# Layjins/Spider

Measured on AMD Instinct MI355X. Metric: multimodal responses/sec (text->text+image), higher is better.
Workload: dtype bf16

## Files before the change

### include/spider_hip.h

```cpp
#ifndef SPIDER_HIP_H
#define SPIDER_HIP_H
#define SPIDER_ABI_VERSION 4

#ifdef __cplusplus
extern "C" {
#endif

int spider_abi_version(void);
const char* spider_target_arch(void);
const char* spider_last_error(void);


int spider_embed_bf16(const void* table, const int* ids, void* out, int rows, int H, int V, void* stream);

int spider_rmsnorm_bf16(const void* x, const void* res, const void* w, void* y, void* res_out, int rows, int H,
                        float eps, void* stream);

int spider_gemv_bf16(const void* W, const void* x, void* out, const void* bias, const void* res, const void* norm_w,
                     float eps, int B, int N, int K, void* stream);

int spider_gemv_swiglu_bf16(const void* W_gate_up, const void* x, void* out, const void* norm_w, float eps, int B,
                            int I, int K, void* stream);

int spider_lm_head_nparts(int V);
// ... 14 lines not shown
int spider_beam_partial_bf16(const void* logits, float* ws_ms, float* ws_val, int* ws_tok, int rows, int V, int C, int nslice,
                             void* stream);
int spider_beam_select_f32(const float* ws_ms, const float* ws_val, const int* ws_tok, float* run_scores, const int* eos_ids,
                           const int* n_eos, const int* n_hist, float* trace_score, int* trace_beam, int* trace_tok, int cap,
                           int* src_beam, int* next_ids, int B, int K, int V, int C, int nslice, void* stream);
int spider_kv_row_gather_bf16(void* k_cache, void* v_cache, void* k_tmp, void* v_tmp, const int* src_beam, const int* kv_beg,
                              const int* kv_end, int K, int R, int layers, int rows_alloc, int n_kv, int T, int d, void* stream);

int spider_sample_partial_bf16(const void* logits, const void* seen, const void* ban, const float* penalty, const int* min_new,
                               const int* eos_ids, const int* n_eos, const int* n_hist, const int* top_k, float* ws_val,
                               int* ws_tok, int rows, int V, int nslice, void* stream);
int spider_sample_select_f32(const float* ws_val, const int* ws_tok, const float* temperature, const float* top_p, const int* top_k,
                             const void* seed, const int* row0, const int* n_hist, int* next_ids, int* cand_tok, float* cand_p,
                             int* n_keep, float* u, int rows, int V, int nslice, void* stream);

int spider_rope_kv_append_bf16(const void* qkv, const int* pos, const int* slot, const float* cos_sin, void* q_out,
                               void* k_cache, void* v_cache, int B, int S, int n_q, int n_kv, int d, int T_max,
                               void* stream);
int spider_rope_kv_append_mrope_bf16(const void* qkv, const int* pos3, const int* slot, const float* cos_sin, void* q_out,
                                     void* k_cache, void* v_cache, int B, int S, int n_q, int n_kv, int d, int T_max,
                                     int sec_t, int sec_h, void* stream);

int spider_attn_decode_bf16(const void* q, const void* k_cache, const void* v_cache, const int* kv_beg,
                            const int* kv_end, void* out, void* ws_o, void* ws_ml, int B, int n_q, int n_kv, int d,
                            int T_max, float scale, int nsplit, void* stream);

int spider_attn_decode_fused_bf16(const void* qkv, const int* pos, const float* cos_sin, void* k_cache, void* v_cache,
                                  const int* kv_beg, const int* kv_end, void* out, void* ws_o, void* ws_ml,
                                  int* counters, int B, int n_q, int n_kv, int d, int T_max, float scale, int nsplit,
                                  void* stream);
int spider_set_attn_inline(int on);
int spider_set_gemv_sched(int sched);
int spider_set_ws_inlaunch(int on);

int spider_gemv_fm_bf16(const void* Wfm, const void* x, void* out, const void* bias, const void* res, int B, int N, int K,
                        int fold_rmsnorm, float eps, void* stream);
int spider_gemv_swiglu_fm_bf16(const void* Wfm_gate_up, const void* x, void* out, int B, int I, int K, int fold_rmsnorm, float eps,
                               void* stream);
int spider_lm_head_argmax_fm_bf16(const void* Wfm, const void* x, int* out_ids, void* logits, void* ws_val, void* ws_idx, int B,
                                  int V, int K, int fold_rmsnorm, float eps, void* stream);
int spider_lm_head_argmax_fm_proc_bf16(const void* Wfm, const void* x, int* out_ids, void* logits, void* ws_val, void* ws_idx,
                                       const void* seen, const void* ban, const float* penalty, const int* min_new,
                                       const int* eos_ids, const int* n_eos, const int* n_hist, int B, int V, int K,
                                       int fold_rmsnorm, float eps, void* stream);


int spider_gemm_bf16(const void* A, const void* W, void* C, void* C32, const void* bias, const void* res,
                     const void* rowbias, int rows_per_group, int M, int N, int K, int lda, int ldc, int act,
                     float out_scale, int w_tiled, const float* res32, float* c32d, void* ws, long ws_bytes, void* stream);

int spider_gemm_ln_bf16(const void* A, const void* Wf, void* C, const float* colsum, const float* colbias, const void* res,
                        int M, int N, int K, int ldc, int act, float eps, int w_tiled, void* ws, long ws_bytes, void* stream);

int spider_xattn_fused_bf16(const void* x, const void* mq_fm, const void* mo_fm, const float* colsum, const float* colbias,
                            const void* bias_o, void* out, int B2, int n_tok, int C, int heads, int n_keys, float eps,
                            const float* x32, float* out32, void* stream);

int spider_conv2d_nhwc_bf16(const void* x, const void* w, void* y, const void* bias, const void* res,
                            const void* rowbias, int B, int Hin, int Win, int Cin, int Cout, int ks, int stride,
                            int pad, int ups, float out_scale, int w_tiled, const float* res32, float* c32d, void* ws, long ws_bytes, void* stream);

int spider_conv_nhwc_ex_bf16(const void* x, const void* w, void* y, const void* bias, const void* res,
                             const void* rowbias, int B, int Hin, int Win, int Cin, int Cout, int kh, int kw, int stride,
                             int pad_h, int pad_w, int dil, int up_h, int up_w, int act, float act_param,
                             float out_scale, int w_tiled, const float* res32, float* c32d, void* ws, long ws_bytes, void* stream);

// ... 181 lines not shown
```

### spider_amd/csrc/capi.cpp

```cpp
#include <string.h>

static thread_local char g_err[512] = "";

extern "C" {

void spider_set_error(const char* msg) {
    strncpy(g_err, msg ? msg : "", sizeof(g_err) - 1);
    g_err[sizeof(g_err) - 1] = 0;
}

const char* spider_last_error(void) { return g_err; }

int spider_abi_version(void) { return 4; }

const char* spider_target_arch(void) { return "gfx950"; }

int g_spider_ws_inlaunch = -1;

int spider_set_ws_inlaunch(int on) {
    const int prev = g_spider_ws_inlaunch;
    g_spider_ws_inlaunch = on ? 1 : 0;
    return prev;
}

}
```

### spider_amd/csrc/common.hpp

```cpp
#pragma once
#include <hip/hip_runtime.h>
#include <stdint.h>

namespace spider {

typedef uint16_t bf16_t;

typedef __attribute__((ext_vector_type(4))) float f32x4;
typedef __attribute__((ext_vector_type(16))) float f32x16;
typedef __attribute__((ext_vector_type(8))) short bf16x8;
typedef __attribute__((ext_vector_type(4))) short bf16x4;

typedef __attribute__((ext_vector_type(4))) uint32_t u32x4;
typedef __attribute__((ext_vector_type(2))) uint32_t u32x2;

__device__ __forceinline__ float bf16_to_f32(bf16_t v) {
    return __uint_as_float(((uint32_t)v) << 16);
}
__device__ __forceinline__ float bf16lo_to_f32(uint32_t packed) {
    return __uint_as_float(packed << 16);
}
__device__ __forceinline__ float bf16hi_to_f32(uint32_t packed) {
    return __uint_as_float(packed & 0xffff0000u);
}
typedef __bf16 hw_bf16x2 __attribute__((ext_vector_type(2)));
typedef float hw_f32x2 __attribute__((ext_vector_type(2)));
__device__ __forceinline__ bf16_t f32_to_bf16(float f) {
    return __builtin_bit_cast(bf16_t, (__bf16)f);
}
__device__ __forceinline__ uint32_t pack_bf16x2(float lo, float hi) {
    const hw_f32x2 v = {lo, hi};
    return __builtin_bit_cast(uint32_t, __builtin_convertvector(v, hw_bf16x2));
}

typedef uint16_t h16_t;
// ... 64 lines not shown
__device__ __forceinline__ float wave_max(float v) {
#pragma unroll
    for (int o = 32; o > 0; o >>= 1) v = fmaxf(v, __shfl_xor(v, o, 64));
    return v;
}

template <int NW>
__device__ __forceinline__ float block_sum(float v, float* red) {
    v = wave_sum(v);
    const int lane = threadIdx.x & 63, w = threadIdx.x >> 6;
    __syncthreads();
    if (lane == 0) red[w] = v;
    __syncthreads();
    float t = 0.f;
#pragma unroll
    for (int i = 0; i < NW; ++i) t += red[i];
    return t;
}

__device__ __forceinline__ float silu_f(float x) { return x * __builtin_amdgcn_rcpf(1.f + __expf(-x)); }
__device__ __forceinline__ float erf_fast(float x) {
    const float ax = fabsf(x);
    const float t = __builtin_amdgcn_rcpf(fmaf(0.3275911f, ax, 1.f));
    float p = fmaf(1.061405429f, t, -1.453152027f);
    p = fmaf(p, t, 1.421413741f);
    p = fmaf(p, t, -0.284496736f);
    p = fmaf(p, t, 0.254829592f);
    const float e = 1.f - p * t * __expf(-ax * ax);
    return copysignf(e, x);
}
__device__ __forceinline__ float gelu_erf_f(float x) { return 0.5f * x * (1.f + erf_fast(x * 0.70710678118654752f)); }
__device__ __forceinline__ float quick_gelu_f(float x) { return x * __builtin_amdgcn_rcpf(1.f + __expf(-1.702f * x)); }

__device__ __forceinline__ int xcd_remap(int bid, int nwg) {
    const int q = nwg >> 3, r = nwg & 7, xcd = bid & 7, idx = bid >> 3;
    const int base = (xcd < r) ? xcd * (q + 1) : r * (q + 1) + (xcd - r) * q;
    return base + idx;
}

}

template <typename F>
inline void raise_dynamic_lds(F* fn, int bytes, unsigned& done_mask) {
    int dev = 0;
    (void)hipGetDevice(&dev);
    const unsigned bit = 1u << (dev & 31);
    if (!(done_mask & bit)) {
        (void)hipFuncSetAttribute(reinterpret_cast<const void*>(fn), hipFuncAttributeMaxDynamicSharedMemorySize, bytes);
        done_mask |= bit;
    }
}

extern "C" void spider_set_error(const char* msg);
extern "C" int g_spider_ws_inlaunch;
#define SPIDER_CHECK(cond, msg)            \
    do {                                   \
        if (!(cond)) {                     \
            spider_set_error(msg);         \
            return -1;                     \
        }                                  \
    } while (0)
#define SPIDER_LAUNCH_OK()                                        \
    do {                                                          \
        hipError_t e__ = hipGetLastError();                       \
        if (e__ != hipSuccess) {                                  \
            spider_set_error(hipGetErrorString(e__));             \
            return -2;                                            \
        }                                                         \
    } while (0)
```

### spider_amd/csrc/gemm.hip

```cpp
#include "common.hpp"
#include <stdlib.h>
#include <stdio.h>
#include <type_traits>

using namespace spider;

namespace {

constexpr int BK = 64;
constexpr int LDS_STRIDE = BK;

struct GemmArgs {
    const h16_t* A;
    const h16_t* W;
    h16_t* C;
    const h16_t* bias;
    const h16_t* res;
    const h16_t* rowbias;
    float* C32;
    const float* res32;
    float* c32d;
    float* ws;
    int M, N, K, lda, ldc;
    uint32_t a_bytes, w_bytes;
    uint32_t c_bytes, rb_bytes;
    int rows_per_group;
    int act;
    float act_param;
    int geglu;
    float out_scale;
    int splits, kt_per_split;
    int conv, Hin, Win, Cin, Hout, Wout, kh, kw, stride, pad_h, pad_w, dil, ups, lim_h, lim_w, cin64;
    int kcm;
    int hbits;
    int dbg;
    int epi_lds;
    int n_fast;
    int w_tiled;
    const float* ln_colsum;
    const float* ln_bias;
    float ln_eps;
    const float2* ln_rows;
    float* gn_part;
    int gn_G, gn_cpg, gn_cr;
    const float* gna_part;
    const h16_t* gna_gamma;
    const h16_t* gna_beta;
    int gna_nchunk, gna_G, gna_hw;
    float gna_eps;
    int ws_ncb, ws_cpb, ws_rows;
    unsigned* ws_cnt;
    int a32;
};

__device__ __forceinline__ float apply_act(const GemmArgs& p, float v) {
    if (p.act == 1) return silu_f(v);
    if (p.act == 2) return gelu_erf_f(v);
    if (p.act == 3) return quick_gelu_f(v);
    if (p.act == 5) return v > 0.f ? v : v * p.act_param;
    if (p.act == 6) return fmaxf(v, 0.f);
    if (p.act == 7) return tanhf(v);
    return v;
}

__device__ __forceinline__ uint32_t w_row_byte(const GemmArgs& p, int n) {
    const uint32_t nk = (uint32_t)((p.K + BK - 1) / BK);
    return p.w_tiled ? ((uint32_t)(n >> 6) * nk * 8192u + (uint32_t)(n & 63) * 128u) : (uint32_t)n * (uint32_t)p.K * 2u;
}
__device__ __forceinline__ uint32_t w_tile_step(const GemmArgs& p) { return p.w_tiled ? 8192u : (uint32_t)(BK * 2); }

// ... 385 lines not shown
        const int m = mb + i * 16 + (lane & 15);
        if (m >= p.M) continue;
#pragma unroll
        for (int j = 0; j < NT; ++j) {
            const int n = nb + j * 16 + (lane >> 4) * 4;
            if (n >= p.N) continue;
            float v[4] = {acc[i][j][0], acc[i][j][1], acc[i][j][2], acc[i][j][3]};
            if (p.splits > 1) {
                float* dst = p.ws + ((size_t)split * p.M + m) * p.N + n;
                if (n + 3 < p.N) *reinterpret_cast<f32x4*>(dst) = f32x4{v[0], v[1], v[2], v[3]};
                else for (int e = 0; e < 4 && n + e < p.N; ++e) dst[e] = v[e];
            } else {
                epilogue_store<EPI>(p, m, n, v);
            }
        }
    }
}

template <int BM, int BN, bool CONV, int EPI, bool LN = false, bool GNA = false, bool A32 = false>
__global__ __launch_bounds__(256, 2) void gemm_kernel(GemmArgs p) {
    constexpr bool GEGLU = EPI == 2;
    extern __shared__ __attribute__((aligned(16))) char smem[];
    h16_t* lds = reinterpret_cast<h16_t*>(smem);
    constexpr int TILE_ELEMS = ((A32 ? 2 : 1) * BM + BN) * LDS_STRIDE;
    constexpr uint32_t AE = A32 ? 4u : 2u;
    constexpr int MT = BM / 32, NT = BN / 32;
    constexpr int AC = BM / 32, WC = BN / 32;

    const int tid = threadIdx.x, lane = tid & 63, wave = tid >> 6;
    const int wm = wave >> 1, wn = wave & 1;

    const int ncols = GEGLU ? 2 * p.N : p.N;
    const int tiles_m = (p.M + BM - 1) / BM, tiles_n = (ncols + BN - 1) / BN;
    const int bid = xcd_remap(blockIdx.x, tiles_m * tiles_n);
    const int tm = p.n_fast ? bid / tiles_n : bid % tiles_m, tn = p.n_fast ? bid % tiles_n : bid / tiles_m;
    const int m0 = tm * BM, n0 = tn * BN;
    const int split = blockIdx.y;

    const int chunk = tid & 7;
    const int lrow = tid >> 3;
    const __amdgpu_buffer_rsrc_t rsrc_a = __builtin_amdgcn_make_buffer_rsrc(const_cast<h16_t*>(p.A), 0, p.a_bytes, 0x00020000);
    const __amdgpu_buffer_rsrc_t rsrc_w = __builtin_amdgcn_make_buffer_rsrc(const_cast<h16_t*>(p.W), 0, p.w_bytes, 0x00020000);
    uint32_t a_base[AC], a_inv[AC];
    uint32_t a_lin[AC];
    uint32_t a_hb[AC];
    int a_oy[AC], a_ox[AC];
    uint32_t w_base[WC], w_inv[WC];
#pragma unroll
    for (int i = 0; i < AC; ++i) {
        const int m = m0 + lrow + 32 * i;
        const bool ok = m < p.M;
        const int mc = ok ? m : 0;
        a_inv[i] = ok ? 0u : 0xFFFFFFFFu;
        if (CONV) {
            const int hw = p.Hout * p.Wout;
            const int b = mc / hw, rem = mc % hw;
            a_oy[i] = (rem / p.Wout) * p.stride - p.pad_h;
            a_ox[i] = (rem % p.Wout) * p.stride - p.pad_w;
            a_base[i] = (uint32_t)b * (uint32_t)(p.Hin * p.Win * p.Cin) * AE;
            a_lin[i] = a_base[i] + (uint32_t)(a_oy[i] * p.Win + a_ox[i]) * (uint32_t)p.Cin * AE;
            a_hb[i] = 0u;
            if (p.hbits) {
                a_lin[i] += chunk * 8u * AE;
                {
                    uint32_t hb = 0u;
                    for (int ky = 0; ky < p.kh; ++ky)
                        for (int kx = 0; kx < p.kw; ++kx) {
                            const int iy = a_oy[i] + ky * p.dil, ix = a_ox[i] + kx * p.dil;
// ... 322 lines not shown
            const int row = idx / CH, c4 = idx - row * CH;
            const int m = m0 + pass * HR + row, n = n0 + c4 * 4;
            const f32x4 q = *reinterpret_cast<const f32x4*>(T + row * LDT + c4 * 4);
            float v[4] = {q[0], q[1], q[2], q[3]};
            uint32_t rb_row = 0;
            if (p.rowbias) rb_row = (uint32_t)((m < p.M ? m : 0) / p.rows_per_group) * (uint32_t)p.N * 2u;
            epilogue_fast<ACT>(p, er, m, n, rb_row, v);
        }
    }
}

template <int N>
__device__ __forceinline__ void wait_vmcnt() {
    asm volatile("s_waitcnt vmcnt(%0)" ::"n"(N) : "memory");
}

template <int BN, int NS, bool CONV, int EPI, int BM = 128, bool GN = false>
__global__ __launch_bounds__(512, NS == 2 ? 2 : 1) void gemm_dma_kernel(GemmArgs p) {
    static_assert(BM == 128 || BM == 64, "row tile");
    constexpr int ROWS = BM + BN;
    constexpr int STAGE = ROWS * 128;
    constexpr int MT = BM / 64, NT = BN / 32;
    constexpr int AJ = BM / 64;
    constexpr int WP = BN / 8;
    constexpr int WJ = (WP + 7) / 8;
    constexpr bool W_RAGGED = (WP % 8) != 0;
    extern __shared__ __attribute__((aligned(16))) char smem[];
    typedef __attribute__((address_space(3))) void* lds_ptr_t;

    const int tid = threadIdx.x, lane = tid & 63;
    const int wave = __builtin_amdgcn_readfirstlane(tid >> 6);
    const int wm = wave >> 1, wn = wave & 1;
    const int tiles_m = (p.M + BM - 1) / BM, tiles_n = (p.N + BN - 1) / BN;
    const int bid = xcd_remap(blockIdx.x, tiles_m * tiles_n);
    const int tm = p.n_fast ? bid / tiles_n : bid % tiles_m, tn = p.n_fast ? bid % tiles_n : bid / tiles_m;
    const int m0 = tm * BM, n0 = tn * BN;
    const int split = blockIdx.y;

    const __amdgpu_buffer_rsrc_t rsrc_a = __builtin_amdgcn_make_buffer_rsrc(const_cast<h16_t*>(p.A), 0, p.a_bytes, 0x00020000);
    const __amdgpu_buffer_rsrc_t rsrc_w = __builtin_amdgcn_make_buffer_rsrc(const_cast<h16_t*>(p.W), 0, p.w_bytes, 0x00020000);

    const int prow = lane >> 3, slot = lane & 7;
    uint32_t a_base[AJ], a_inv[AJ], a_gch[AJ], a_lin[AJ];
    uint32_t a_hb[AJ];
    int a_oy[AJ], a_ox[AJ];
    uint32_t w_base[WJ], w_inv[WJ], w_gch[WJ];
#pragma unroll
    for (int j = 0; j < AJ; ++j) {
        const int R = (j * 8 + wave) * 8 + prow;
        const int m = m0 + R;
        const bool ok = m < p.M;
        const int mc = ok ? m : 0;
        a_gch[j] = (uint32_t)(slot ^ ((R >> 1) & 7));
        a_inv[j] = ok ? 0u : 0xFFFFFFFFu;
        if (CONV) {
            const int hw = p.Hout * p.Wout;
            const int b = mc / hw, rem = mc % hw;
            a_oy[j] = (rem / p.Wout) * p.stride - p.pad_h;
            a_ox[j] = (rem % p.Wout) * p.stride - p.pad_w;
            a_base[j] = (uint32_t)b * (uint32_t)(p.Hin * p.Win * p.Cin) * 2u;
            a_lin[j] = a_base[j] + (uint32_t)(a_oy[j] * p.Win + a_ox[j]) * (uint32_t)p.Cin * 2u;
            a_hb[j] = 0u;
            if (p.hbits) {
                a_lin[j] += a_gch[j] * 16u;
                {
                    uint32_t hb = 0u;
                    for (int ky = 0; ky < p.kh; ++ky)
                        for (int kx = 0; kx < p.kw; ++kx) {
// ... 149 lines not shown
        constexpr int NCH = BM / 64, WPC = 4 / NCH;
        const int cpg = p.gn_cpg, gpt = BN / cpg;
        for (int t = tid; t < NCH * gpt; t += 512) {
            const int c = t / gpt, gi = t - c * gpt;
            const int col0 = gi * cpg, ncol = n0 + col0;
            const int mrow = m0 + c * 64;
            if (ncol >= p.N || mrow >= p.M) continue;
            const int wn_ = col0 / (BN / 2), cw = col0 - wn_ * (BN / 2);
            float ss = 0.f, qq = 0.f;
            for (int w = 0; w < WPC; ++w) {
                const float2* src = cols + ((c * WPC + w) * 2 + wn_) * (BN / 2) + cw;
                for (int k = 0; k < cpg; ++k) { ss += src[k].x; qq += src[k].y; }
            }
            float* dst = p.gn_part + ((size_t)(mrow >> 6) * p.gn_G + (ncol / cpg)) * 2;
            dst[0] = ss;
            dst[1] = qq;
        }
    }
}

template <bool CONV, int EPI, bool LN = false>
__global__ __launch_bounds__(512, 1) void gemm_p8_kernel(GemmArgs p) {
    constexpr bool GEGLU = EPI == 2;
    constexpr int HT = 128 * 128;
    constexpr int KT_BYTES = 4 * HT;
    extern __shared__ __attribute__((aligned(16))) char smem[];
    typedef __attribute__((address_space(3))) void* lds_ptr_t;

    const int tid = threadIdx.x, lane = tid & 63;
    const int wave = __builtin_amdgcn_readfirstlane(tid >> 6);
    const int wr = wave >> 2, wc = wave & 3;
    const int ncols = GEGLU ? 2 * p.N : p.N;
    const int tiles_m = (p.M + 255) / 256, tiles_n = (ncols + 255) / 256;
    const int bid = xcd_remap(blockIdx.x, tiles_m * tiles_n);
    const int tm = p.n_fast ? bid / tiles_n : bid % tiles_m, tn = p.n_fast ? bid % tiles_n : bid / tiles_m;
    const int m0 = tm * 256, n0 = tn * 256;
    const int split = blockIdx.y;

    const __amdgpu_buffer_rsrc_t rsrc_a = __builtin_amdgcn_make_buffer_rsrc(const_cast<h16_t*>(p.A), 0, p.a_bytes, 0x00020000);
    const __amdgpu_buffer_rsrc_t rsrc_w = __builtin_amdgcn_make_buffer_rsrc(const_cast<h16_t*>(p.W), 0, p.w_bytes, 0x00020000);

    const int prow = lane >> 3, slot = lane & 7;
    uint32_t a_base[2][2], a_inv[2][2], a_lin[2][2], w_base[2][2], w_inv[2][2], gch[2];
    uint32_t a_hb[2][2] = {{0u, 0u}, {0u, 0u}};
    int a_oy[2][2], a_ox[2][2];
#pragma unroll
    for (int j = 0; j < 2; ++j) {
        const int R = (j * 8 + wave) * 8 + prow;
        gch[j] = (uint32_t)(slot ^ ((R >> 1) & 7));
#pragma unroll
        for (int h = 0; h < 2; ++h) {
            const int m = m0 + h * 128 + R;
            const bool okm = m < p.M;
            const int mc = okm ? m : 0;
            a_inv[h][j] = okm ? 0u : 0xFFFFFFFFu;
            if (CONV) {
                const int hw = p.Hout * p.Wout;
                const int b = mc / hw, rem = mc % hw;
                a_oy[h][j] = (rem / p.Wout) * p.stride - p.pad_h;
                a_ox[h][j] = (rem % p.Wout) * p.stride - p.pad_w;
                a_base[h][j] = (uint32_t)b * (uint32_t)(p.Hin * p.Win * p.Cin) * 2u;
                a_lin[h][j] = a_base[h][j] + (uint32_t)(a_oy[h][j] * p.Win + a_ox[h][j]) * (uint32_t)p.Cin * 2u;
                if (p.hbits) {
                    a_lin[h][j] += gch[j] * 16u;
                    uint32_t hb = 0u;
                    for (int ky = 0; ky < p.kh; ++ky)
                        for (int kx = 0; kx < p.kw; ++kx) {
                            const int iy = a_oy[h][j] + ky * p.dil, ix = a_ox[h][j] + kx * p.dil;
// ... 165 lines not shown
        __builtin_amdgcn_s_barrier();
        issue(0, 0, kt + 2, cur);
        __builtin_amdgcn_sched_barrier(0);
        if (wr == 1) wait_vmcnt<4>();
        slot_end();
        mfmas(1, 0);
        if (wr == 0) wait_vmcnt<4>();
        __builtin_amdgcn_s_barrier();
        cur = nxt;
    }
    if (wr == 0) __builtin_amdgcn_s_barrier();
    wait_vmcnt<0>();

    if (GEGLU) {
        geglu_out<8, 2, LN>(p, acc, m0 + wr * 128, (n0 / 2) + wc * 32, lane, p.ln_rows, 0);
        return;
    }
    write_out<8, 4, EPI, LN>(p, acc, m0 + wr * 128, n0 + wc * 64, split, lane, p.ln_rows, 0);
}

template <bool CONV, int EPI>
__global__ __launch_bounds__(512, 1) void gemm_p8h_kernel(GemmArgs p) {
    constexpr int HT = 128 * 128;
    constexpr int KT_BYTES = 3 * HT;
    constexpr int NSTG = 3;
    extern __shared__ __attribute__((aligned(16))) char smem[];
    typedef __attribute__((address_space(3))) void* lds_ptr_t;

    const int tid = threadIdx.x, lane = tid & 63;
    const int wave = __builtin_amdgcn_readfirstlane(tid >> 6);
    const int wr = wave >> 1, wc = wave & 1;
    const int grp = wave >> 2;
    const int tiles_m = (p.M + 255) / 256, tiles_n = (p.N + 127) / 128;
    const int bid = xcd_remap(blockIdx.x, tiles_m * tiles_n);
    const int tm = p.n_fast ? bid / tiles_n : bid % tiles_m, tn = p.n_fast ? bid % tiles_n : bid / tiles_m;
    const int m0 = tm * 256, n0 = tn * 128;
    const int split = blockIdx.y;

    const __amdgpu_buffer_rsrc_t rsrc_a = __builtin_amdgcn_make_buffer_rsrc(const_cast<h16_t*>(p.A), 0, p.a_bytes, 0x00020000);
    const __amdgpu_buffer_rsrc_t rsrc_w = __builtin_amdgcn_make_buffer_rsrc(const_cast<h16_t*>(p.W), 0, p.w_bytes, 0x00020000);

    const int prow = lane >> 3, slot = lane & 7;
    uint32_t a_base[2][2], a_inv[2][2], a_lin[2][2], w_base[2], w_inv[2], gch[2];
    uint32_t a_hb[2][2];
    int a_oy[2][2], a_ox[2][2];
#pragma unroll
    for (int j = 0; j < 2; ++j) {
        const int R = (j * 8 + wave) * 8 + prow;
        gch[j] = (uint32_t)(slot ^ ((R >> 1) & 7));
#pragma unroll
        for (int h = 0; h < 2; ++h) {
            const int m = m0 + h * 128 + R;
            const bool okm = m < p.M;
            const int mc = okm ? m : 0;
            a_inv[h][j] = okm ? 0u : 0xFFFFFFFFu;
            if (CONV) {
                const int hw = p.Hout * p.Wout;
                const int b = mc / hw, rem = mc % hw;
                a_oy[h][j] = (rem / p.Wout) * p.stride - p.pad_h;
                a_ox[h][j] = (rem % p.Wout) * p.stride - p.pad_w;
                a_base[h][j] = (uint32_t)b * (uint32_t)(p.Hin * p.Win * p.Cin) * 2u;
                a_lin[h][j] = a_base[h][j] + (uint32_t)(a_oy[h][j] * p.Win + a_ox[h][j]) * (uint32_t)p.Cin * 2u;
                a_hb[h][j] = 0u;
                if (p.hbits) {
                    a_lin[h][j] += gch[j] * 16u;
                    uint32_t hb = 0u;
                    for (int ky = 0; ky < p.kh; ++ky)
                        for (int kx = 0; kx < p.kw; ++kx) {
// ... 762 lines not shown
        a.ws_cnt = (g_spider_ws_inlaunch && S > 1 && S <= 8 && strips <= 1024) ? reinterpret_cast<unsigned*>(reinterpret_cast<char*>(a.ws) + ws_bytes) : nullptr;
        dim3 grid(strips, S);
        if (a.M <= 128) launch_ws_inst<1, 8, false>(a, grid, st);
        else if (a.ups) launch_ws_inst<4, 2, true>(a, grid, st);
        else launch_ws_inst<4, 2, false>(a, grid, st);
        SPIDER_LAUNCH_OK();
        if (a.ws_cnt) return 0;
        if (a.gn_part && a.splits == 1) a.gn_part = nullptr;
    } else {
    static const int force_tile = env_int("SPIDER_GEMM_TILE"), force_splits = env_int("SPIDER_GEMM_SPLITS");
    const int nk = (a.K + BK - 1) / BK;
    const int ncols = a.geglu ? 2 * a.N : a.N;
    const int t128 = ((a.M + 127) / 128) * ((ncols + 127) / 128);
    const int t64 = ((a.M + 63) / 64) * ((ncols + 63) / 64);
    bool small;
    int splits = 1;
    if (nk >= 44 && t128 >= 24) {
        small = false;
        splits = 768 / t128;
        if (splits < nk / 32) splits = nk / 32;
        if (splits > 8) splits = 8;
        if (splits > nk / 8) splits = nk / 8;
    } else if (t128 >= 320) {
        small = false;
    } else {
        small = true;
        if (t64 < 256 && nk >= 64) {
            splits = (512 + t64 - 1) / t64;
            if (splits > 16) splits = 16;
            if (splits > nk / 4) splits = nk / 4;
        }
    }
    if (force_tile) small = force_tile == 64;
    static const int nfast_env = getenv("SPIDER_GEMM_NFAST") ? atoi(getenv("SPIDER_GEMM_NFAST")) : -1;
    a.n_fast = nfast_env >= 0 ? nfast_env : (a.M > ncols ? 1 : 0);
    int dma_bn = (force_tile == 160 || force_tile == 161 || force_tile == 162) ? 160 : (force_tile == 129 ? 128 : (force_tile == 65 ? 64 : 0));
    bool dma_ns2 = force_tile == 162;
    const int n160 = (a.N + 159) / 160;
    int dma_bm = 128;
    static const int bm64_env = getenv("SPIDER_GEMM_BM64") ? atoi(getenv("SPIDER_GEMM_BM64")) : 1;
    const bool dma_rows = a.conv ? a.M >= 512 : (a.M >= 2048 || (a.M >= 512 && nk >= 64));
    if (!force_tile && !a.geglu && dma_rows && nk >= (a.conv && a.M >= 2048 ? 16 : 40) && n160 * 160 * 25 <= a.N * 27) {
        if (bm64_env && ((a.M + 127) / 128) * n160 <= 160 && a.M >= 1024 && nk < 64) dma_bm = 64;
        const int tdma = ((a.M + dma_bm - 1) / dma_bm) * n160;
        int ds = 1;
        if (nk >= 40) {
            ds = (256 + tdma / 2) / tdma;
            if (ds > 8) ds = 8;
            if (ds > nk / 8) ds = nk / 8;
            if (ds < 1) ds = 1;
        }
        const int blocks = tdma * ds, rounds = (blocks + 255) / 256;
        if (blocks <= 256 || blocks * 100 >= rounds * 256 * 85) {
            dma_bn = 160;
            splits = ds;
        }
    }
    static const int p8_env = getenv("SPIDER_GEMM_P8") ? atoi(getenv("SPIDER_GEMM_P8")) : 1;
    bool use_p8 = false;
    int p8_splits = 1, p8_rounds = 1;
    const bool p8_fused = a.geglu || a.ln_colsum;
    const size_t ln_rows_bytes = (size_t)((a.M + 255) / 256) * 256 * sizeof(float2);
    if (p8_env && !force_tile && !force_splits && nk >= 8 && !(a.geglu && a.conv) &&
        (!a.ln_colsum || (a.ws && ln_rows_bytes <= (size_t)ws_bytes && a.act == 0))) {
        const long t256 = (long)((a.M + 255) / 256) * ((ncols + 255) / 256);
        if ((double)a.M * ncols >= 0.75 * 65536.0 * (double)t256) {
            int s = 1;
            if (t256 < 160 && a.ws && !p8_fused) {
// ... 41 lines not shown
        float best_t = 0.f;
        auto cost = [&](int i, bool with_stream) {
            const long tiles_i = (long)((a.M + cand[i].bm - 1) / cand[i].bm) * ((ncols + cand[i].bn - 1) / cand[i].bn);
            const float stream = (with_stream && i != 4) ? 6.0f * (float)nstream * (float)(cand[i].bm * cand[i].bn) / 20480.f : 0.f;
            float rounds = (float)((tiles_i + cand[i].slots - 1) / cand[i].slots);
            if (i == 4) rounds = 0.5f * (rounds + (float)tiles_i / (float)cand[i].slots);
            return cand[i].pre + rounds * (cand[i].t0 + stream + (float)nk * cand[i].tk);
        };
        for (int i = 0; i < 4; ++i) {
            if (!cand[i].ok) continue;
            const float t = cost(i, false);
            if (best < 0 || t < best_t) { best = i; best_t = t; }
        }
        if (cand[4].ok && (best < 0 || cost(4, true) < cost(best, true))) best = 4;
        use_p8 = best == 0; use_p8h = best == 1;
        dma_bn = (best == 2 || best == 4) ? 160 : 0; dma_bm = 128;
        dma_ns2 = best == 4;
        small = false; splits = 1; p8_splits = 1;
    }
    if (a.gna_part) { use_p8 = use_p8h = false; dma_bn = 0; small = true; splits = 1; }
    if (a.a32) { use_p8 = use_p8h = false; dma_bn = 0; }
    if (use_p8h) { use_p8 = false; splits = 1; dma_bn = 0; }
    if (use_p8) { splits = p8_splits; dma_bn = 0; }
    if (a.ln_colsum) { dma_bn = 0; splits = 1; }
    if (!a.ws || splits < 1 || a.geglu) splits = 1;
    while (splits > 1 && (size_t)splits * a.M * a.N * sizeof(float) > (size_t)ws_bytes) --splits;
    const int tiles = small ? t64 : t128;
    if (force_splits && a.ws && !a.geglu && !a.ln_colsum) {
        splits = force_splits < nk ? force_splits : nk;
        while (splits > 1 && (size_t)splits * a.M * a.N * sizeof(float) > (size_t)ws_bytes) --splits;
    }
    a.kt_per_split = (nk + splits - 1) / splits;
    a.splits = (nk + a.kt_per_split - 1) / a.kt_per_split;
    static const int trace = env_int("SPIDER_GEMM_TRACE");
    if (trace)
        fprintf(stderr, "spider_gemm_dispatch M=%d N=%d K=%d conv=%d(%dx%d s%d ups%d) geglu=%d ln=%d a32=%d -> %s splits=%d\n", a.M, a.N, a.K, a.conv,
                a.kh, a.kw, a.stride, a.ups, a.geglu, a.ln_colsum != nullptr, a.a32,
                use_p8h ? "p8h(256x128)" : use_p8 ? "p8(256x256)" : (dma_bn && !a.geglu) ? (dma_ns2 ? "dma2(128x160, 2 per CU)" : dma_bm == 64 ? "dma(64x160)" : "dma(128x160)")
                                                                   : small ? "reg(64x64)" : "reg(128x128)", a.splits);
    if (use_p8h || (force_tile == 257 && !a.geglu && !a.ln_colsum)) {
        launch_p8h(a, st);
    } else if (use_p8 || (force_tile == 256 && !a.geglu && !a.ln_colsum)) {
        if (a.ln_colsum) {
            a.ln_rows = reinterpret_cast<const float2*>(a.ws);
            ln_row_stats_kernel<<<(a.M + 3) / 4, 256, 0, st>>>(a.A, reinterpret_cast<float2*>(a.ws), a.M, a.K, a.ln_eps);
            SPIDER_LAUNCH_OK();
        }
        launch_p8(a, st);
    } else if (dma_bn && !a.geglu) {
        const int tdma = ((a.M + dma_bm - 1) / dma_bm) * ((a.N + dma_bn - 1) / dma_bn);
        if (a.gn_part && a.splits == 1) { a.gn_cr = 64; if (!(dma_bn == 160 && force_tile != 161 && dma_gn_ok(a))) a.gn_part = nullptr; }
        if (gn_done && a.gn_part && a.splits == 1) *gn_done = 64;
        const bool ns2 = dma_ns2;
        a.epi_lds = epi_lds_env == 2 || (epi_lds_env == 1 && ns2 && (a.res32 || a.c32d));
        if (dma_bn == 64) launch_dma<64, 6>(a, tdma, st);
        else if (ns2) launch_dma<160, 2>(a, tdma, st);
        else if (force_tile == 161) launch_dma<160, 4>(a, tdma, st);
        else if (dma_bn == 160 && dma_bm == 64) launch_dma<160, 4, 64>(a, tdma, st);
        else if (dma_bn == 160) launch_dma<160, 3>(a, tdma, st);
        else launch_dma<128, 4>(a, tdma, st);
    } else if (small) launch_tile<64, 64>(a, tiles, st);
    else launch_tile<128, 128>(a, tiles, st);
    SPIDER_LAUNCH_OK();
    }
    if (a.splits > 1) {
        const int cs = (a.gn_part && a.splits <= 16 && a.gn_cpg > 0 && a.N % a.gn_cpg == 0 && a.N % 4 == 0 && a.M % 16 == 0 && !a.C32 &&
                        (!a.conv || a.rows_per_group % 16 == 0))
                           ? gn_reduce_slab(a.gn_cpg, a.M >= 1024 ? 160 : 80) : 0;
        a.gn_cr = 16;
        if (cs) {
            const int nq = cs / 4;
            const int blocks = (a.M / 16) * ((a.N + cs - 1) / cs);
// ... 256 lines not shown
```

### spider_amd/lib.py

```python
from __future__ import annotations

import ctypes as C
import os
import threading

import torch

_HERE = os.path.dirname(os.path.abspath(__file__))
LIB_PATH = os.path.join(_HERE, "libspider_hip.so")

_lib = None
_lock = threading.Lock()

_vp, _i, _f, _l = C.c_void_p, C.c_int, C.c_float, C.c_long

SIGNATURES = {
    "spider_abi_version": (_i, []),
    "spider_target_arch": (C.c_char_p, []),
    "spider_last_error": (C.c_char_p, []),
    "spider_embed_bf16": (_i, [_vp, _vp, _vp, _i, _i, _i, _vp]),
    "spider_rmsnorm_bf16": (_i, [_vp, _vp, _vp, _vp, _vp, _i, _i, _f, _vp]),
    "spider_gemv_bf16": (_i, [_vp, _vp, _vp, _vp, _vp, _vp, _f, _i, _i, _i, _vp]),
    "spider_gemv_swiglu_bf16": (_i, [_vp, _vp, _vp, _vp, _f, _i, _i, _i, _vp]),
    "spider_lm_head_nparts": (_i, [_i]),
    "spider_decode_advance_i32": (_i, [_vp] * 7 + [_i, _i, _vp]),
    "spider_lm_head_argmax_bf16": (_i, [_vp, _vp, _vp, _f, _vp, _vp, _vp, _vp, _i, _i, _i, _vp]),
    "spider_lm_head_argmax_proc_bf16": (_i, [_vp, _vp, _vp, _f] + [_vp] * 11 + [_i, _i, _i, _vp]),
    "spider_decode_advance_seen_i32": (_i, [_vp] * 8 + [_i, _i, _i, _vp]),
    "spider_token_bitmap_set_i32": (_i, [_vp, _vp, _i, _i, _i, _vp]),
    "spider_beam_partial_bf16": (_i, [_vp] * 4 + [_i] * 4 + [_vp]),
    "spider_beam_select_f32": (_i, [_vp] * 10 + [_i, _vp, _vp] + [_i] * 5 + [_vp]),
    "spider_kv_row_gather_bf16": (_i, [_vp] * 7 + [_i] * 7 + [_vp]),
    "spider_sample_partial_bf16": (_i, [_vp] * 11 + [_i] * 3 + [_vp]),
    "spider_sample_select_f32": (_i, [_vp] * 13 + [_i] * 3 + [_vp]),
    "spider_gemv_fm_bf16": (_i, [_vp, _vp, _vp, _vp, _vp, _i, _i, _i, _i, _f, _vp]),
    "spider_gemv_swiglu_fm_bf16": (_i, [_vp, _vp, _vp, _i, _i, _i, _i, _f, _vp]),
    "spider_lm_head_argmax_fm_bf16": (_i, [_vp, _vp, _vp, _vp, _vp, _vp, _i, _i, _i, _i, _f, _vp]),
    "spider_lm_head_argmax_fm_proc_bf16": (_i, [_vp] * 13 + [_i, _i, _i, _i, _f, _vp]),
    "spider_rope_kv_append_bf16": (_i, [_vp, _vp, _vp, _vp, _vp, _vp, _vp, _i, _i, _i, _i, _i, _i, _vp]),
    "spider_rope_kv_append_mrope_bf16": (_i, [_vp, _vp, _vp, _vp, _vp, _vp, _vp, _i, _i, _i, _i, _i, _i, _i, _i, _vp]),
    "spider_attn_decode_bf16": (_i, [_vp, _vp, _vp, _vp, _vp, _vp, _vp, _vp, _i, _i, _i, _i, _i, _f, _i, _vp]),
    "spider_attn_decode_fused_bf16": (_i, [_vp] * 11 + [_i, _i, _i, _i, _i, _f, _i, _vp]),
    "spider_set_attn_inline": (_i, [_i]),
    "spider_set_gemv_sched": (_i, [_i]),
    "spider_set_ws_inlaunch": (_i, [_i]),
    "spider_gemm_bf16": (_i, [_vp, _vp, _vp, _vp, _vp, _vp, _vp, _i, _i, _i, _i, _i, _i, _i, _f, _i, _vp, _vp, _vp, _l, _vp]),
    "spider_gemm_ln_bf16": (_i, [_vp, _vp, _vp, _vp, _vp, _vp, _i, _i, _i, _i, _i, _f, _i, _vp, _l, _vp]),
    "spider_xattn_fused_bf16": (_i, [_vp, _vp, _vp, _vp, _vp, _vp, _vp, _i, _i, _i, _i, _i, _f, _vp, _vp, _vp]),
    "spider_conv2d_nhwc_bf16": (_i, [_vp, _vp, _vp, _vp, _vp, _vp, _i, _i, _i, _i, _i, _i, _i, _i, _i, _f, _i, _vp, _vp, _vp, _l, _vp]),
    "spider_conv_nhwc_ex_bf16": (_i, [_vp] * 6 + [_i] * 14 + [_f, _f, _i, _vp, _vp, _vp, _l, _vp]),
    "spider_attn_bf16": (_i, [_vp, _vp, _vp, _vp] + [_l] * 12 + [_i] * 6 + [_f, _i, _i, _vp, _vp, _i, _i, _vp]),
    "spider_story_key_lists_i32": (_i, [_vp, _i, _i, _i, _i, _i, _i, _vp, _vp, _vp]),
    "spider_attn_keylist_bf16": (_i, [_vp, _vp, _vp, _vp] + [_l] * 12 + [_i] * 6 + [_f, _vp, _i, _vp, _i, _vp]),
    "spider_attn_varlen_bf16": (_i, [_vp, _vp, _vp, _vp, _l, _l, _l, _l, _i, _i, _i, _i, _f, _vp, _i, _vp]),
    "spider_rope_rows_bf16": (_i, [_vp, _vp, _l, _i, _i, _i, _vp]),
    "spider_groupnorm_nchunk": (_i, [_i]),
    "spider_groupnorm_nhwc_bf16": (_i, [_vp, _vp, _vp, _vp, _vp, _i, _i, _i, _i, _f, _i, _vp]),
    "spider_groupnorm_cat_nhwc_bf16": (_i, [_vp] * 7 + [_i, _i, _i, _i, _i, _f, _i, _vp]),
    "spider_conv_nhwc_gn_bf16": (_i, [_vp] * 6 + [_i] * 14 + [_f, _f, _i, _vp, _vp, _vp, _l, _vp] + [_vp, _i, _vp]),
    "spider_groupnorm_stats_nhwc_bf16": (_i, [_vp, _vp, _i, _i, _i, _i, _i, _vp]),
    "spider_groupnorm_apply_nhwc_bf16": (_i, [_vp, _vp, _i, _vp, _vp, _vp, _i, _i, _i, _i, _f, _i, _vp]),
    "spider_gemm_gn_in_bf16": (_i, [_vp, _vp, _vp, _vp, _i, _i, _i, _i, _i, _vp, _i, _vp, _vp, _i, _f, _i, _vp, _vp]),
    "spider_layernorm_bf16": (_i, [_vp, _vp, _vp, _vp, _i, _i, _f, _vp]),
    "spider_geglu_bf16": (_i, [_vp, _vp, _i, _i, _vp]),
    "spider_swiglu_bf16": (_i, [_vp, _vp, _i, _i, _vp]),
    "spider_concat_channels_bf16": (_i, [_vp, _vp, _vp, _l, _i, _i, _vp]),
    "spider_act_bf16": (_i, [_vp, _vp, _l, _i, _vp]),
    "spider_add_bf16": (_i, [_vp, _vp, _vp, _l, _vp]),
    "spider_act_ex_bf16": (_i, [_vp, _vp, _l, _i, _f, _vp]),
    "spider_add_scaled_bf16": (_i, [_vp, _vp, _vp, _l, _f, _vp]),
    "spider_axpby_bf16": (_i, [_vp, _vp, _vp, _l, _f, _f, _vp]),
    "spider_mean_tokens_bf16": (_i, [_vp, _vp, _i, _i, _i, _vp]),
    "spider_moe_combine_bf16": (_i, [_vp, _i, _vp, _i, _vp, _i, _l, _vp]),
    "spider_col2im1d_f32_bf16": (_i, [_vp, _vp, _vp, _i, _i, _i, _i, _i, _i, _vp]),
    "spider_l2_normalize_rows_bf16": (_i, [_vp, _vp, _i, _i, _f, _vp]),
    "spider_conv2d_small_cin_bf16": (_i, [_vp, _vp, _vp, _vp, _i, _i, _i, _i, _i, _i, _vp]),
    "spider_conv2d_small_cout_bf16": (_i, [_vp, _vp, _vp, _vp, _vp, _i, _i, _i, _i, _i, _i, _vp]),
    "spider_latent_to_nhwc_bf16": (_i, [_vp, _vp, _i, _i, _i, _i, _f, _vp]),
# ... 66 lines not shown
```

### spider_amd/ops.py

```python
from __future__ import annotations

import ctypes as C
import math
from typing import Optional

import torch

from . import lib as _lib

BF16 = torch.bfloat16
ACT = {None: 0, "none": 0, "silu": 1, "gelu": 2, "quick_gelu": 3, "geglu": 4, "leaky_relu": 5, "relu": 6, "tanh": 7, "swiglu": 8,
       "geglu_exact": 9}
GLU_ACTS = ("geglu", "swiglu", "geglu_exact")


def _stream() -> int:
    return torch.cuda.current_stream().cuda_stream


_WS = {}
WS_BYTES = 64 << 20
WS_TAIL = 4096


# ... 66 lines not shown
    t = getattr(W, "_spider_tiled", None)
    tag = (W._version, W.data_ptr())
    if t is None or getattr(W, "_spider_tiled_tag", None) != tag:
        if torch.cuda.is_current_stream_capturing():
            if t is not None:
                raise RuntimeError("a marked weight was modified in place and is first used again under stream capture: call "
                                   "ops.prebuild_tiled() (or run one eager pass) before capturing")
            return None
        t = tile_weight64(W.reshape(W.shape[0], -1))
        W._spider_tiled, W._spider_tiled_tag = t, tag
    return t


def prebuild_tiled(weights, max_rows: int = 64 << 20) -> int:
    n = 0
    for W in weights:
        if getattr(W, "_spider_weight", False) and W.ndim >= 2 and W.numel() <= max_rows:
            t = _tiled(W, 1)
            n += 0 if t is None else t.numel() * t.element_size()
    return n


WS_ENABLE = _os.environ.get("SPIDER_WS", "1") != "0"
WS_INLAUNCH = _os.environ.get("SPIDER_WS_INLAUNCH", "1") != "0"
WS_MAX_M = int(_os.environ.get("SPIDER_WS_MAX_M", "128"))


def set_ws_inlaunch(on: bool) -> bool:
    global WS_INLAUNCH
    prev = WS_INLAUNCH
    _lib.load().spider_set_ws_inlaunch(int(bool(on)))
    WS_INLAUNCH = bool(on)
    return prev


def repack_fm_conv(W: torch.Tensor) -> torch.Tensor:
    N, kh, kw, Cin = W.shape
    assert kh == 3 and kw == 3 and Cin % 32 == 0
    Np = (N + 31) // 32 * 32
    if Np != N:
        W = torch.cat([W, torch.zeros(Np - N, kh, kw, Cin, dtype=W.dtype, device=W.device)], 0)
    return W.reshape(Np // 16, 16, 9, Cin // 32, 4, 8).permute(0, 3, 2, 4, 1, 5).contiguous().view(Np // 16, (Cin // 32) * 9, 64, 8)


def _ws_eligible(B, Hin, Win, Cin, Cout, kh, kw, stride, pad, dil, up_size, Ho, Wo, act) -> bool:
    if not WS_ENABLE or (kh, kw) != (3, 3) or stride != 1 or dil != 1 or tuple(pad) != (1, 1) or Cin % 32 or Cout % 4 or act:
        return False
    M, rows = B * Ho * Wo, B * Hin * Win
    if M > WS_MAX_M:
        return False
    if M <= 128:
        return rows <= 128 and up_size is None
    return M <= 512 and rows <= 512


def _wsfm(W: torch.Tensor):
    if not getattr(W, "_spider_weight", False):
        return None
    t = getattr(W, "_spider_fm", None)
    tag = (W._version, W.data_ptr())
    if t is None or getattr(W, "_spider_fm_tag", None) != tag:
        if torch.cuda.is_current_stream_capturing():
            if t is not None:
                raise RuntimeError("a marked weight was modified in place and is first used again under stream capture")
            return None
        t = repack_fm_conv(W)
# ... 1136 lines not shown
```

Before: 1.996.

## Assign GEMM tiles to XCDs in 2D blocks chosen by a traffic cost model

Replaces the 1D XCD remap plus m-fast/n-fast order with a 2D partition: each of the 8 XCDs gets an r×c block of output tiles, with (r,c,inner) picked by a host cost model that estimates A and W bytes each XCD must fetch. The aim is to cut duplicated A/W reads across XCD-private L2 caches for larger GEMMs and convs. It adds per-block integer loops in the kernel prologue. The model is a heuristic and may choose worse orders for some shapes.

```diff
diff --git a/include/spider_hip.h b/include/spider_hip.h
--- a/include/spider_hip.h
+++ b/include/spider_hip.h
@@ -70,6 +70,9 @@
 int spider_set_attn_inline(int on);
 int spider_set_gemv_sched(int sched);
 int spider_set_ws_inlaunch(int on);
+int spider_set_gemm_xcd2d(int mode);
+int spider_gemm_tile_order(int tiles_m, int tiles_n, int r, int c, int inner, int* tm, int* tn);
+int spider_gemm_xcd_shape(int M, int ncols, int K, int cin, int taps, int kcm, int a_rows, int bm, int bn, int model, int* shape);
 
 int spider_gemv_fm_bf16(const void* Wfm, const void* x, void* out, const void* bias, const void* res, int B, int N, int K,
                         int fold_rmsnorm, float eps, void* stream);
diff --git a/spider_amd/csrc/capi.cpp b/spider_amd/csrc/capi.cpp
--- a/spider_amd/csrc/capi.cpp
+++ b/spider_amd/csrc/capi.cpp
@@ -1,4 +1,6 @@
 #include <string.h>
+
+#include "tile_order.hpp"
 
 static thread_local char g_err[512] = "";
 
@@ -23,4 +25,31 @@
     return prev;
 }
 
+int g_spider_gemm_xcd2d = -1;
+
+int spider_set_gemm_xcd2d(int mode) {
+    const int prev = g_spider_gemm_xcd2d;
+    g_spider_gemm_xcd2d = (mode >= 0 && mode <= 9) ? mode : 1;
+    return prev;
 }
+
+int spider_gemm_tile_order(int tiles_m, int tiles_n, int r, int c, int inner, int* tm, int* tn) {
+    if (tiles_m < 1 || tiles_n < 1 || r < 1 || c < 1 || r * c != 8 || !tm || !tn || (long)tiles_m * tiles_n >= (1l << 31)) {
+        spider_set_error("gemm_tile_order: need tiles_m, tiles_n >= 1, r * c = 8 and both outputs");
+        return -1;
+    }
+    for (int b = 0; b < tiles_m * tiles_n; ++b) spider::xcd_tile_2d(b, tiles_m, tiles_n, r, c, inner ? 1 : 0, tm[b], tn[b]);
+    return 0;
+}
+
+int spider_gemm_xcd_shape(int M, int ncols, int K, int cin, int taps, int kcm, int a_rows, int bm, int bn, int model, int* shape) {
+    if (M < 1 || ncols < 1 || K < 1 || bm < 1 || bn < 1 || !shape || (cin > 0 && (taps < 1 || K != taps * cin))) {
+        spider_set_error("gemm_xcd_shape: need a non-empty problem, tile sizes, the output array, and K = taps * cin for a conv");
+        return -1;
+    }
+    const spider::XcdShape s = model ? spider::xcd_choose_shape(M, ncols, K, cin > 0, cin, taps, kcm, 2, bm, bn, a_rows > 0 ? a_rows : M) : spider::xcd_legacy_shape(M, ncols);
+    shape[0] = s.r; shape[1] = s.c; shape[2] = s.inner;
+    return 0;
+}
+
+}
diff --git a/spider_amd/csrc/common.hpp b/spider_amd/csrc/common.hpp
--- a/spider_amd/csrc/common.hpp
+++ b/spider_amd/csrc/common.hpp
@@ -1,6 +1,7 @@
 #pragma once
 #include <hip/hip_runtime.h>
 #include <stdint.h>
+#include "tile_order.hpp"
 
 namespace spider {
 
@@ -131,11 +132,6 @@
 __device__ __forceinline__ float gelu_erf_f(float x) { return 0.5f * x * (1.f + erf_fast(x * 0.70710678118654752f)); }
 __device__ __forceinline__ float quick_gelu_f(float x) { return x * __builtin_amdgcn_rcpf(1.f + __expf(-1.702f * x)); }
 
-__device__ __forceinline__ int xcd_remap(int bid, int nwg) {
-    const int q = nwg >> 3, r = nwg & 7, xcd = bid & 7, idx = bid >> 3;
-    const int base = (xcd < r) ? xcd * (q + 1) : r * (q + 1) + (xcd - r) * q;
-    return base + idx;
-}
 
 }
 
@@ -151,6 +147,7 @@
 }
 
 extern "C" void spider_set_error(const char* msg);
+extern "C" int g_spider_gemm_xcd2d;
 extern "C" int g_spider_ws_inlaunch;
 #define SPIDER_CHECK(cond, msg)            \
     do {                                   \
diff --git a/spider_amd/csrc/gemm.hip b/spider_amd/csrc/gemm.hip
--- a/spider_amd/csrc/gemm.hip
+++ b/spider_amd/csrc/gemm.hip
@@ -36,6 +36,7 @@
     int dbg;
     int epi_lds;
     int n_fast;
+    int xcd_r, xcd_c;
     int w_tiled;
     const float* ln_colsum;
     const float* ln_bias;
@@ -487,8 +488,8 @@
 
     const int ncols = GEGLU ? 2 * p.N : p.N;
     const int tiles_m = (p.M + BM - 1) / BM, tiles_n = (ncols + BN - 1) / BN;
-    const int bid = xcd_remap(blockIdx.x, tiles_m * tiles_n);
-    const int tm = p.n_fast ? bid / tiles_n : bid % tiles_m, tn = p.n_fast ? bid % tiles_n : bid / tiles_m;
+    int tm, tn;
+    xcd_tile_2d(blockIdx.x, tiles_m, tiles_n, p.xcd_r, p.xcd_c, p.n_fast, tm, tn);
     const int m0 = tm * BM, n0 = tn * BN;
     const int split = blockIdx.y;
 
@@ -877,8 +878,8 @@
     const int wave = __builtin_amdgcn_readfirstlane(tid >> 6);
     const int wm = wave >> 1, wn = wave & 1;
     const int tiles_m = (p.M + BM - 1) / BM, tiles_n = (p.N + BN - 1) / BN;
-    const int bid = xcd_remap(blockIdx.x, tiles_m * tiles_n);
-    const int tm = p.n_fast ? bid / tiles_n : bid % tiles_m, tn = p.n_fast ? bid % tiles_n : bid / tiles_m;
+    int tm, tn;
+    xcd_tile_2d(blockIdx.x, tiles_m, tiles_n, p.xcd_r, p.xcd_c, p.n_fast, tm, tn);
     const int m0 = tm * BM, n0 = tn * BN;
     const int split = blockIdx.y;
 
@@ -1094,8 +1095,8 @@
     const int wr = wave >> 2, wc = wave & 3;
     const int ncols = GEGLU ? 2 * p.N : p.N;
     const int tiles_m = (p.M + 255) / 256, tiles_n = (ncols + 255) / 256;
-    const int bid = xcd_remap(blockIdx.x, tiles_m * tiles_n);
-    const int tm = p.n_fast ? bid / tiles_n : bid % tiles_m, tn = p.n_fast ? bid % tiles_n : bid / tiles_m;
+    int tm, tn;
+    xcd_tile_2d(blockIdx.x, tiles_m, tiles_n, p.xcd_r, p.xcd_c, p.n_fast, tm, tn);
     const int m0 = tm * 256, n0 = tn * 256;
     const int split = blockIdx.y;
 
@@ -1327,8 +1328,8 @@
     const int wr = wave >> 1, wc = wave & 1;
     const int grp = wave >> 2;
     const int tiles_m = (p.M + 255) / 256, tiles_n = (p.N + 127) / 128;
-    const int bid = xcd_remap(blockIdx.x, tiles_m * tiles_n);
-    const int tm = p.n_fast ? bid / tiles_n : bid % tiles_m, tn = p.n_fast ? bid % tiles_n : bid / tiles_m;
+    int tm, tn;
+    xcd_tile_2d(blockIdx.x, tiles_m, tiles_n, p.xcd_r, p.xcd_c, p.n_fast, tm, tn);
     const int m0 = tm * 256, n0 = tn * 128;
     const int split = blockIdx.y;
 
@@ -2157,8 +2158,6 @@
         }
     }
     if (force_tile) small = force_tile == 64;
-    static const int nfast_env = getenv("SPIDER_GEMM_NFAST") ? atoi(getenv("SPIDER_GEMM_NFAST")) : -1;
-    a.n_fast = nfast_env >= 0 ? nfast_env : (a.M > ncols ? 1 : 0);
     int dma_bn = (force_tile == 160 || force_tile == 161 || force_tile == 162) ? 160 : (force_tile == 129 ? 128 : (force_tile == 65 ? 64 : 0));
     bool dma_ns2 = force_tile == 162;
     const int n160 = (a.N + 159) / 160;
@@ -2266,12 +2265,29 @@
     }
     a.kt_per_split = (nk + splits - 1) / splits;
     a.splits = (nk + a.kt_per_split - 1) / a.kt_per_split;
+    {
+        const bool k_p8h = use_p8h || (force_tile == 257 && !a.geglu && !a.ln_colsum);
+        const bool k_p8 = !k_p8h && (use_p8 || (force_tile == 256 && !a.geglu && !a.ln_colsum));
+        const bool k_dma = !k_p8h && !k_p8 && dma_bn && !a.geglu;
+        const int bm = (k_p8h || k_p8) ? 256 : k_dma ? (dma_bn == 160 ? dma_bm : 128) : small ? 64 : 128;
+        const int bn = k_p8h ? 128 : k_p8 ? 256 : k_dma ? dma_bn : small ? 64 : 128;
+        const int cols = (k_p8h || k_dma) ? a.N : ncols;
+        static const int nfast_env = getenv("SPIDER_GEMM_NFAST") ? atoi(getenv("SPIDER_GEMM_NFAST")) : -1;
+        if (g_spider_gemm_xcd2d < 0) g_spider_gemm_xcd2d = getenv("SPIDER_GEMM_XCD2D") ? atoi(getenv("SPIDER_GEMM_XCD2D")) : 1;
+        const int mode = g_spider_gemm_xcd2d;
+        XcdShape xs = xcd_legacy_shape(a.M, ncols);
+        if (nfast_env >= 0) { xs.r = nfast_env ? 8 : 1; xs.c = nfast_env ? 1 : 8; xs.inner = nfast_env ? 1 : 0; }
+        else if (mode >= 2 && mode <= 9) { xs.r = 8 >> ((mode - 2) >> 1); xs.c = 8 / xs.r; xs.inner = (mode - 2) & 1; }
+        else if (mode == 1) xs = xcd_choose_shape(a.M, cols, a.K, a.conv, a.Cin, a.kh * a.kw, a.kcm, a.a32 ? 4 : 2, bm, bn,
+                                                 a.conv ? (long)(a.M / (a.Hout * a.Wout)) * a.Hin * a.Win : a.M);
+        a.xcd_r = xs.r; a.xcd_c = xs.c; a.n_fast = xs.inner;
+    }
     static const int trace = env_int("SPIDER_GEMM_TRACE");
     if (trace)
-        fprintf(stderr, "spider_gemm_dispatch M=%d N=%d K=%d conv=%d(%dx%d s%d ups%d) geglu=%d ln=%d a32=%d -> %s splits=%d\n", a.M, a.N, a.K, a.conv,
+        fprintf(stderr, "spider_gemm_dispatch M=%d N=%d K=%d conv=%d(%dx%d s%d ups%d) geglu=%d ln=%d a32=%d -> %s splits=%d xcd=%dx%d%c\n", a.M, a.N, a.K, a.conv,
                 a.kh, a.kw, a.stride, a.ups, a.geglu, a.ln_colsum != nullptr, a.a32,
                 use_p8h ? "p8h(256x128)" : use_p8 ? "p8(256x256)" : (dma_bn && !a.geglu) ? (dma_ns2 ? "dma2(128x160, 2 per CU)" : dma_bm == 64 ? "dma(64x160)" : "dma(128x160)")
-                                                                   : small ? "reg(64x64)" : "reg(128x128)", a.splits);
+                                                                   : small ? "reg(64x64)" : "reg(128x128)", a.splits, a.xcd_r, a.xcd_c, a.n_fast ? 'n' : 'm');
     if (use_p8h || (force_tile == 257 && !a.geglu && !a.ln_colsum)) {
         launch_p8h(a, st);
     } else if (use_p8 || (force_tile == 256 && !a.geglu && !a.ln_colsum)) {
diff --git a/spider_amd/csrc/tile_order.hpp b/spider_amd/csrc/tile_order.hpp
--- /dev/null
+++ b/spider_amd/csrc/tile_order.hpp
@@ -0,0 +1,70 @@
+#pragma once
+
+#if defined(__HIPCC__)
+#define SPIDER_HD __host__ __device__ inline __attribute__((always_inline))
+#else
+#define SPIDER_HD inline
+#endif
+
+namespace spider {
+
+SPIDER_HD int xcd_remap(int bid, int nwg) {
+    const int q = nwg >> 3, r = nwg & 7, xcd = bid & 7, idx = bid >> 3;
+    const int base = (xcd < r) ? xcd * (q + 1) : r * (q + 1) + (xcd - r) * q;
+    return base + idx;
+}
+
+SPIDER_HD void xcd_tile_2d(int bid, int tiles_m, int tiles_n, int r, int c, int inner, int& tm, int& tn) {
+    const int L = xcd_remap(bid, tiles_m * tiles_n);
+    if (r > tiles_m) r = tiles_m;
+    if (c > tiles_n) c = tiles_n;
+    if (r < 1) r = 1;
+    if (c < 1) c = 1;
+    int i = r - 1;
+    while (i > 0 && (i * tiles_m / r) * tiles_n > L) --i;
+    const int m0 = i * tiles_m / r, h = (i + 1) * tiles_m / r - m0;
+    const int off = L - m0 * tiles_n;
+    int j = c - 1;
+    while (j > 0 && h * (j * tiles_n / c) > off) --j;
+    const int n0 = j * tiles_n / c, w = (j + 1) * tiles_n / c - n0;
+    const int o = off - h * n0;
+    if (inner) { tm = m0 + o / w; tn = n0 + o % w; }
+    else       { tm = m0 + o % h; tn = n0 + o / h; }
+}
+
+struct XcdShape { int r, c, inner; };
+
+SPIDER_HD XcdShape xcd_legacy_shape(long M, long ncols) {
+    XcdShape s;
+    if (M > ncols) { s.r = 8; s.c = 1; s.inner = 1; }
+    else           { s.r = 1; s.c = 8; s.inner = 0; }
+    return s;
+}
+
+SPIDER_HD XcdShape xcd_choose_shape(long M, long ncols, long K, int conv, long Cin, int taps, int kcm, int esize, int bm, int bn,
+                                    long a_rows) {
+    const XcdShape legacy = xcd_legacy_shape(M, ncols);
+    const long small = 2l << 20;
+    const long a_bytes = (conv ? a_rows * Cin * (kcm ? 1 : taps) : M * K) * esize;
+    const long w_bytes = ncols * K * esize;
+    const int tiles_m = (int)((M + bm - 1) / bm), tiles_n = (int)((ncols + bn - 1) / bn);
+    XcdShape best = legacy;
+    double best_cost = -1.0;
+    for (int k = -1; k < 4; ++k) {
+        XcdShape s;
+        if (k < 0) s = legacy;
+        else { s.r = 8 >> k; s.c = 1 << k; s.inner = 0; }
+        const int r = s.r < tiles_m ? s.r : tiles_m, c = s.c < tiles_n ? s.c : tiles_n;
+        const double ca = a_bytes <= small ? (double)a_bytes : (double)a_bytes / r;
+        const double cw = w_bytes <= small ? (double)w_bytes : (double)w_bytes / c;
+        const double cost = ca + cw;
+        if (best_cost < 0.0 || cost < best_cost) {
+            best_cost = cost;
+            best = s;
+            if (k >= 0) best.inner = s.r == 8 ? 1 : (s.c == 8 ? 0 : ((double)w_bytes / c <= (double)a_bytes / r ? 1 : 0));
+        }
+    }
+    return best;
+}
+
+}
diff --git a/spider_amd/lib.py b/spider_amd/lib.py
--- a/spider_amd/lib.py
+++ b/spider_amd/lib.py
@@ -44,6 +44,9 @@
     "spider_set_attn_inline": (_i, [_i]),
     "spider_set_gemv_sched": (_i, [_i]),
     "spider_set_ws_inlaunch": (_i, [_i]),
+    "spider_set_gemm_xcd2d": (_i, [_i]),
+    "spider_gemm_tile_order": (_i, [_i, _i, _i, _i, _i, _vp, _vp]),
+    "spider_gemm_xcd_shape": (_i, [_i] * 10 + [_vp]),
     "spider_gemm_bf16": (_i, [_vp, _vp, _vp, _vp, _vp, _vp, _vp, _i, _i, _i, _i, _i, _i, _i, _f, _i, _vp, _vp, _vp, _l, _vp]),
     "spider_gemm_ln_bf16": (_i, [_vp, _vp, _vp, _vp, _vp, _vp, _i, _i, _i, _i, _i, _f, _i, _vp, _l, _vp]),
     "spider_xattn_fused_bf16": (_i, [_vp, _vp, _vp, _vp, _vp, _vp, _vp, _i, _i, _i, _i, _i, _f, _vp, _vp, _vp]),
diff --git a/spider_amd/ops.py b/spider_amd/ops.py
--- a/spider_amd/ops.py
+++ b/spider_amd/ops.py
@@ -122,6 +122,24 @@
     _lib.load().spider_set_ws_inlaunch(int(bool(on)))
     WS_INLAUNCH = bool(on)
     return prev
+
+
+def set_gemm_xcd2d(mode: int) -> int:
+    return int(_lib.load().spider_set_gemm_xcd2d(int(mode)))
+
+
+def gemm_tile_order(tiles_m: int, tiles_n: int, r: int, c: int, inner: int):
+    n = tiles_m * tiles_n
+    tm, tn = (C.c_int * n)(), (C.c_int * n)()
+    _lib.call("spider_gemm_tile_order", tiles_m, tiles_n, r, c, inner, C.cast(tm, C.c_void_p), C.cast(tn, C.c_void_p))
+    return list(zip(tm, tn))
+
+
+def gemm_xcd_shape(M: int, ncols: int, K: int, bm: int, bn: int, cin: int = 0, taps: int = 1, kcm: bool = True, model: bool = True,
+                   a_rows: int = 0):
+    s = (C.c_int * 3)()
+    _lib.call("spider_gemm_xcd_shape", M, ncols, K, cin, taps, int(kcm), a_rows, bm, bn, int(model), C.cast(s, C.c_void_p))
+    return tuple(s)
 
 
 def repack_fm_conv(W: torch.Tensor) -> torch.Tensor:
```

Result: no change. 1.994 (median of 2 runs) (-0.1%).
